# Hcyand/recommender_system

Hardware: AMD Instinct MI355X
Metric: CTR forward samples/sec @ batch 4096, 26 sparse×1e7 vocab, dim 16; %HBM roofline (higher is better)
Workload: dtype f32

## Files before the change

### recommender_system_amd/csrc/embed_fm_body.hpp

```cpp
#pragma once
#include "embed_fm.hpp"
#include "mlp_tower.hpp"

namespace rs {

#ifdef RS_DIAG_STAMPS
#define RS_STAMP(i)                                                                          \
  do {                                                                                       \
    __builtin_amdgcn_sched_barrier(0);                                                       \
    if (a.dbg && lane == 0)                                                                  \
      a.dbg[((int64_t)blockIdx.x * NW + w) * 16 + (i)] = __builtin_amdgcn_s_memrealtime();  \
    __builtin_amdgcn_sched_barrier(0);                                                       \
  } while (0)
#define RS_USE(x) asm volatile("" ::"v"(x))
#else
#define RS_STAMP(i) \
  do {              \
  } while (0)
#define RS_USE(x) \
  do {            \
  } while (0)
#endif

template <int KV, int NT, int NW, int KIND, bool TW, int MC = 0, bool PF = false, bool KA = false, int FC = 0,
          int KFMC = 0, int NDC = -1, bool PL = false>
__device__ __forceinline__ void embed_fm_body(const EmbedFmArgs& a, const MlpArgs* tw, const int tile,
                                              const FieldMeta* km = nullptr) {
  const int aF = FC > 0 ? FC : a.F;
  const int akfm = KFMC > 0 ? KFMC : a.kfm;
  const int and_ = NDC >= 0 ? NDC : a.nd;
  constexpr int MAXC0 = MC > 0 ? MC : 128 / (NW * KV);
  constexpr int MAXC = MAXC0 < 1 ? 1 : (MAXC0 > 8 ? 8 : MAXC0);
  typedef Ids<(KIND >= 3) ? 0 : KIND> I;
  constexpr bool OWNER = KIND == 4;
  __shared__ float cs[NW][16][NT * 16 + 1];
  __shared__ float qs[NW][16];

  const int lane = threadIdx.x & 63;
  const int w = __builtin_amdgcn_readfirstlane(threadIdx.x >> 6);
  const int s = lane & 15;
  const int kk = lane >> 4;
  const int64_t bt = (int64_t)tile * 16 + s;
  const bool valid = bt < a.batch;
  const int64_t b = bt < a.batch ? bt : a.batch - 1;
  const int d = and_ + aF * a.k;
  float w0v = (OWNER || PL) ? 0.f : a.w0[0];

  floatx4 ac[NT][4];
#pragma unroll
  for (int nt = 0; nt < NT; ++nt)
#pragma unroll
    for (int c = 0; c < 4; ++c) ac[nt][c] = floatx4{0.f, 0.f, 0.f, 0.f};
  float qn = 0.f;
  bool bad = false;

  if constexpr (!PL) {
    asm volatile("" ::"s"(a.ids), "s"(a.id_stride), "s"(a.dense), "s"(a.dense_stride), "s"(a.nd), "s"(a.table),
                 "s"(a.offs), "s"(a.vocab), "s"(aF), "s"(a.k), "s"(a.prep), "s"(akfm));
    asm volatile("" ::"s"(a.batch), "s"(a.DB), "s"(a.dense_rec), "s"(a.field_rec), "s"(a.field_base), "s"(a.x_out),
                 "s"(a.logit), "s"(a.w0), "s"(a.err));
  }
  RS_STAMP(0);
  RS_USE(b);
  RS_STAMP(5);
  if constexpr (TW) {
    const MlpArgs& a = *tw;
    MLP_STAMP(0);
  }
  extern __shared__ float tsm[];
  __shared__ float fmlog[TW ? 16 : 1];
  floatx4 ring[TW ? MLP_R : 1];
  const int xrs = TW ? tw->rs : 0;
  if constexpr (TW) {
    mlp_first_fill<NW>(*tw, ring);
    float* par = tsm + 32 * tw->rs + NW * 256;
    for (int i = threadIdx.x; i < tw->ptot; i += NW * 64) par[i] = tw->prep[tw->wtot + i];
    const int d0 = aF * a.k + and_, padw = tw->Kp[0] - d0;
    for (int i = threadIdx.x; i < 16 * padw; i += NW * 64) {
      const int r = i / padw;
      tsm[r * xrs + d0 + (i - r * padw)] = 0.f;
    }
  }
  const bool dense_small = KA || a.DB <= NW;
  const int dw = NW - 1 - w;
  const bool has_dense = dense_small && dw < a.DB;
  float dx = 0.f, dn = 0.f, drec[NT];
#pragma unroll
  for (int nt = 0; nt < NT; ++nt) drec[nt] = 0.f;
  auto load_dense = [&]() {
    if (has_dense) {
      const int e = 4 * dw + kk;
      dx = a.dense[b * a.dense_stride + (e < and_ ? e : 0)];
      const float* rec = a.prep + (int64_t)dw * a.dense_rec;
#pragma unroll
      for (int nt = 0; nt < NT; ++nt) drec[nt] = rec[nt * 64 + lane];
      dn = rec[NT * 64 + kk];
    }
  };
  constexpr int FMAX = 128;
  __shared__ typename I::raw_t lid[16][FMAX];
  __shared__ int64_t lmeta[2][FMAX];
#ifdef RS_DIAG_STAMPS
  const bool coop = !KA && !OWNER && (KIND != 3) && aF <= FMAX && !(a.ablate & 16);
#else
  const bool coop = !KA && !OWNER && (KIND != 3) && aF <= FMAX;
#endif
  if (coop) {
    const int64_t b0 = (int64_t)tile * 16;
    for (int t = threadIdx.x; t < 16 * aF; t += NW * 64) {
      const int ss = t / aF, c = t - ss * aF;
      const int64_t bb = b0 + ss < a.batch ? b0 + ss : a.batch - 1;
      const auto idv = I::load(a.ids, bb * a.id_stride + c);
#ifdef RS_DIAG_STAMPS
      RS_USE(idv);
      RS_STAMP(8);
#endif
      lid[ss][c] = idv;
    }
    if constexpr (!OWNER) {
      for (int t = threadIdx.x; t < 2 * aF; t += NW * 64) {
        const int c = t < aF ? t : t - aF;
        lmeta[t < aF ? 0 : 1][c] = t < aF ? a.offs[c] : a.vocab[c];
      }
    }
  }
  struct Pass {
    int cj[MAXC];
    bool ok[MAXC];
    typename I::raw_t rid[MAXC];
    int64_t off[MAXC], voc[MAXC];
    int64_t row[MAXC];
    Chunk<KV> xs[MAXC];
    Chunk<KV> bw[MAXC][NT];
    float nrm[MAXC][KV];
  };
  auto issue_b = [&](int cg, Pass& P) {
#pragma unroll
    for (int j = 0; j < MAXC; ++j) {
      const int c = cg + j * NW + w;
      P.cj[j] = c < aF ? c : aF - 1;
      const float* rec = a.prep + a.field_base + (int64_t)P.cj[j] * a.field_rec;
#pragma unroll
      for (int nt = 0; nt < NT; ++nt) {
#ifdef RS_DIAG_STAMPS
        if (a.ablate & 2) { P.bw[j][nt].zero(); P.bw[j][nt].v[0] = (float)P.cj[j]; continue; }
#endif
        if (nt * 16 + s <= akfm) P.bw[j][nt].load(rec + (int64_t)(nt * 64 + lane) * KV);
        else P.bw[j][nt].zero();
      }
    }
  };
  auto norms = [&](Pass& P) {
#pragma unroll
    for (int j = 0; j < MAXC; ++j)
#pragma unroll
      for (int tp = 0; tp < KV; ++tp) {
        float sq = 0.f;
#pragma unroll
        for (int nt = 0; nt < NT; ++nt) {
          const float bv = nt * 16 + s < akfm ? P.bw[j][nt].v[tp] : 0.f;
          sq = fmaf(bv, bv, sq);
        }
        P.nrm[j][tp] = row16_sum(sq);
      }
  };
  const int wv = threadIdx.x >> 6;
  auto fetch_ids = [&](int cg, Pass& P) {
    int64_t* offc = P.off;
    int64_t* vocc = P.voc;
#pragma unroll
    for (int j = 0; j < MAXC; ++j) {
      if constexpr (KIND != 3) {
        if (OWNER) {
          offc[j] = 0;
          vocc[j] = a.owner_rows;
          P.rid[j] = coop ? lid[s][P.cj[j]] : I::load(a.ids, b * a.id_stride + P.cj[j]);
        } else if (coop) {
          offc[j] = lmeta[0][P.cj[j]];
          vocc[j] = lmeta[1][P.cj[j]];
          P.rid[j] = lid[s][P.cj[j]];
        } else if constexpr (KA) {
          offc[j] = km->off[P.cj[j]];
          vocc[j] = km->voc[P.cj[j]];
          P.rid[j] = I::load(a.ids, b * a.id_stride + P.cj[j]);
        } else {
          const int cv = min(cg + j * NW + wv, aF - 1);
          offc[j] = a.offs[cv];
          vocc[j] = a.vocab[cv];
          P.rid[j] = I::load(a.ids, b * a.id_stride + P.cj[j]);
        }
      }
    }
    if (cg == 0 && !coop && aF > 0) load_dense();
  };
  auto decode_rows = [&](int cg, Pass& P) {
    if (cg == 0) RS_STAMP(6);
    else RS_STAMP(10);
#pragma unroll
    for (int j = 0; j < MAXC; ++j) {
      if constexpr (KIND == 3) {
        P.row[j] = b * aF + P.cj[j];
        P.ok[j] = true;
      } else {
        int64_t id;
        P.ok[j] = I::decode(P.rid[j], P.voc[j], id);
        P.row[j] = P.off[j] + id;
      }
    }
    RS_USE(P.row[MAXC - 1]);
    if (cg == 0) RS_STAMP(1);
    else RS_STAMP(11);
  };
  auto load_rows = [&](int cg, Pass& P) {
#pragma unroll
    for (int j = 0; j < MAXC; ++j) {
#ifdef RS_DIAG_STAMPS
      if ((a.ablate & 8) && cg + j * NW + w >= aF) { P.xs[j].zero(); continue; }
#endif
      P.xs[j].load_nt(a.table + P.row[j] * a.k + KV * kk);
    }
  };
  auto issue_rows = [&](int cg, Pass& P, bool fetched) {
    if (!fetched) fetch_ids(cg, P);
    decode_rows(cg, P);
    load_rows(cg, P);
  };
  auto consume = [&](int cg, Pass& P) {
    RS_USE(P.xs[MAXC - 1].v[KV - 1]);
    RS_USE(P.bw[MAXC - 1][0].v[KV - 1]);
    if (cg == 0) RS_STAMP(2);
    else RS_STAMP(12);
#pragma unroll
    for (int j = 0; j < MAXC; ++j) {
      const bool live = cg + j * NW + w < aF;
      if constexpr (OWNER) bad |= live && !P.ok[j] && P.rid[j] != -1;
      else bad |= live && !P.ok[j];
      const bool use = live && P.ok[j];
#pragma unroll
      for (int tp = 0; tp < KV; ++tp) {
        const float xv = use ? P.xs[j].v[tp] : 0.f;
#pragma unroll
        for (int nt = 0; nt < NT; ++nt) {
#ifdef RS_DIAG_STAMPS
          if (a.ablate & 1) { ac[nt][0][0] += xv * P.bw[j][nt].v[tp]; continue; }
#endif
          ac[nt][tp & 3] = mfma16x16x4(xv, P.bw[j][nt].v[tp], ac[nt][tp & 3]);
        }
        qn = fmaf(xv * xv, P.nrm[j][tp], qn);
      }
      if constexpr (TW) {
        if (live) {
          float* xo = tsm + s * xrs + P.cj[j] * a.k + KV * kk;
#pragma unroll
          for (int tp = 0; tp < KV; ++tp) xo[tp] = P.ok[j] ? P.xs[j].v[tp] : 0.f;
        }
      } else if (!KA && a.x_out && live && valid) {
        float* xo = a.x_out + b * d + and_ + P.cj[j] * a.k + KV * kk;
#pragma unroll
        for (int tp = 0; tp < KV; ++tp) xo[tp] = P.ok[j] ? P.xs[j].v[tp] : 0.f;
      }
    }
    RS_USE(ac[0][0][0]);
    if (cg == 0) RS_STAMP(13);
    else RS_STAMP(14);
  };
  auto has_pass = [&](int cg) { return cg < aF && !(MAXC == 1 && cg + w >= aF); };
  constexpr int PS = NW * MAXC;
  constexpr bool PRE = PF && KV * MAXC * NT <= 8;
  auto late_args = [&]() {
    if constexpr (PL) {
      w0v = a.w0[0];
      asm volatile("" ::"s"(a.k), "s"(a.logit), "s"(a.w0), "s"(a.err));
    }
  };
  Pass P0, P1;
  if (PRE) {
    if (has_pass(0)) issue_b(0, P0);
    if (has_pass(PS)) issue_b(PS, P1);
  }
  if (aF == 0 || coop) load_dense();
  if (coop) __syncthreads();
  RS_STAMP(9);
  if (PRE) {
    const bool one = has_pass(0), two = one && has_pass(PS);
    if (one) {
      fetch_ids(0, P0);
      if (two) fetch_ids(PS, P1);
    } else if (!coop && aF > 0) {
      load_dense();
    }
    late_args();
    if (one) {
      issue_rows(0, P0, true);
      if constexpr (PL) asm volatile("" ::"s"(w0v));
      norms(P0);
      if (two) norms(P1);
      if (two) decode_rows(PS, P1);
      consume(0, P0);
      if (two) {
        load_rows(PS, P1);
        consume(PS, P1);
        for (int cg = 2 * PS; !KA && has_pass(cg); cg += PS) {
          issue_b(cg, P0);
          issue_rows(cg, P0, false);
          norms(P0);
          consume(cg, P0);
        }
      }
    }
  } else {
    late_args();
    for (int cg = 0; has_pass(cg); cg += PS) {
      issue_b(cg, P0);
      issue_rows(cg, P0, false);
      norms(P0);
      consume(cg, P0);
    }
  }

  if (has_dense) {
    const int e = 4 * dw + kk;
    dx = e < and_ ? dx : 0.f;
#pragma unroll
    for (int nt = 0; nt < NT; ++nt) ac[nt][0] = mfma16x16x4(dx, drec[nt], ac[nt][0]);
    qn = fmaf(dx * dx, dn, qn);
    if constexpr (TW) {
      if (e < and_) tsm[s * xrs + aF * a.k + e] = dx;
    } else if (!KA && a.x_out && valid && e < and_) {
      a.x_out[b * d + e] = dx;
    }
  }
  if (!dense_small) {
    for (int t = w; t < a.DB; t += NW) {
      const int e = 4 * t + kk;
      const float xv = a.dense[b * a.dense_stride + (e < and_ ? e : 0)];
      const float x = e < and_ ? xv : 0.f;
      const float* rec = a.prep + (int64_t)t * a.dense_rec;
#pragma unroll
      for (int nt = 0; nt < NT; ++nt) ac[nt][0] = mfma16x16x4(x, rec[nt * 64 + lane], ac[nt][0]);
      qn = fmaf(x * x, rec[NT * 64 + kk], qn);
      if constexpr (TW) {
        if (e < and_) tsm[s * xrs + aF * a.k + e] = x;
      } else if (a.x_out && valid && e < and_) {
        a.x_out[b * d + e] = x;
      }
    }
  }
  floatx4 acc[NT];
#pragma unroll
  for (int nt = 0; nt < NT; ++nt)
#pragma unroll
    for (int i = 0; i < 4; ++i) acc[nt][i] = (ac[nt][0][i] + ac[nt][1][i]) + (ac[nt][2][i] + ac[nt][3][i]);
  RS_USE(acc[0][0]);
  RS_STAMP(3);
  if (__any(bad && valid) && lane == 0) flag_error(a.err);

#ifdef RS_DIAG_STAMPS
  if (a.ablate & 4) {
    if (w == 0 && kk == 0 && b < a.batch) a.logit[b] = acc[0][0] + acc[0][1] + qn;
    return;
  }
#endif
#pragma unroll
  for (int nt = 0; nt < NT; ++nt)
#pragma unroll
    for (int r = 0; r < 4; ++r) cs[w][kk * 4 + r][nt * 16 + s] = acc[nt][r];
  qn += __shfl_xor(qn, 16);
  qn += __shfl_xor(qn, 32);
  if (lane < 16) qs[w][lane] = qn;
  __syncthreads();
  RS_STAMP(7);
  constexpr int NC = NT * 16;
  if (threadIdx.x < 16 * NC) {
    const int smp = threadIdx.x / NC, col = threadIdx.x % NC;
    float v = 0.f;
#pragma unroll
    for (int ww = 0; ww < NW; ++ww) v += cs[ww][smp][col];
    float t = col < akfm ? v * v : 0.f;
    if (col < NW) t -= qs[col][smp];
    float lin = col == akfm ? v : 0.f;
    t = row16_sum(t);
    lin = row16_sum(lin);
    if constexpr (NT == 2) {
      t += __shfl_xor(t, 16);
      lin += __shfl_xor(lin, 16);
    }
    const int64_t bb = (int64_t)tile * 16 + smp;
    if constexpr (OWNER) {
      float q = col < NW ? qs[col][smp] : 0.f;
      q = row16_sum(q);
      if constexpr (NT == 2) q += __shfl_xor(q, 16);
      if (bb < a.batch) {
        float* rec = a.logit + bb * a.pstride;
        if (col <= akfm) rec[col] = v;
        if (col == 0) rec[akfm + 1] = q;
        else if (akfm + 1 + col < a.pw) rec[akfm + 1 + col] = 0.f;
      }
      return;
    }
    const float fm = (lin + w0v) + 0.5f * t;
    if (col == 0 && bb < a.batch && a.logit) a.logit[bb] = fm;
    if constexpr (TW) {
      if (col == 0) fmlog[smp] = fm;
    }
  }
  RS_STAMP(4);
  if constexpr (TW) {
    {
      const MlpArgs& a = *tw;
      MLP_STAMP(1);
    }
    mlp_tower_tile<NW>(*tw, tsm, (int64_t)tile * 16, ring, fmlog);
  }
}

struct EmbedFmCold {
  float* logit;
  const float* w0;
  int* err;
  int F, k, nd, kfm;
  const int64_t* offs;
  const int64_t* vocab;
  float* x_out;
  int DB;
  int64_t dense_rec, field_rec, field_base;
  int64_t owner_rows;
  int pw;
  int64_t pstride;
  unsigned long long* dbg;
  int ablate;
};

static inline EmbedFmCold cold_args(const EmbedFmArgs& a) {
  return EmbedFmCold{a.logit, a.w0,        a.err,       a.F,          a.k,          a.nd, a.kfm,     a.offs, a.vocab,
                     a.x_out, a.DB,        a.dense_rec, a.field_rec,  a.field_base, a.owner_rows,    a.pw,   a.pstride,
                     a.dbg,   a.ablate};
}

template <int KV, int NT, int FC, int KFMC, int NDC>
__device__ __forceinline__ EmbedFmArgs hot_cold_args(const float* prep, const void* ids, int64_t id_stride,
                                                     int64_t batch, const float* dense, int64_t dense_stride,
                                                     const float* table, const EmbedFmCold& c) {
  EmbedFmArgs a;
  a.ids = ids;
  a.id_stride = id_stride;
  a.dense = dense;
  a.dense_stride = dense_stride;
  a.nd = c.nd;
  a.table = table;
  a.offs = c.offs;
  a.vocab = c.vocab;
  a.F = c.F;
  a.k = c.k;
  a.prep = prep;
  a.w0 = c.w0;
  a.kfm = c.kfm;
  a.logit = c.logit;
  a.x_out = c.x_out;
  a.batch = batch;
  a.err = c.err;
  if constexpr (FC > 0) {
    constexpr FmGeom G = fm_geom(NDC, FC, 4 * KV, KFMC);
    static_assert(G.mfma && G.KV == KV && G.NT == NT, "specialised shape: not this instantiation's geometry");
    a.DB = G.DB;
    a.dense_rec = G.dense_rec;
    a.field_rec = G.field_rec;
    a.field_base = G.field_base;
  } else {
    a.DB = c.DB;
    a.dense_rec = c.dense_rec;
    a.field_rec = c.field_rec;
    a.field_base = c.field_base;
  }
  a.owner_rows = c.owner_rows;
  a.pw = c.pw;
  a.pstride = c.pstride;
  a.dbg = c.dbg;
  a.ablate = c.ablate;
  return a;
}

}
```

Before: 713.0 million.

## Restructure FM embed body: early second-pass row loads, wide LDS reduce, permlane swaps

Several independent tweaks to the fused embedding+FM kernel. A compile-time row stride is used when the field count is fixed. The second pass's row offsets are precomputed and its table loads are issued behind a scheduling barrier before the first pass is consumed, to overlap gather latency. Dense loading moves out of fetch_ids when prefetching, and the per-field bias loads become unconditional in the KA path. The cross-wave LDS reduction layout is transposed so each output reads contiguous floatx4 vectors, and qn shuffles are replaced with permlane16/32 swaps. Together these add code complexity and raise register pressure and LDS size.

Measured after the change: 751.6 million, median of 6. 1.05x the previous value.

```diff
diff --git a/recommender_system_amd/csrc/embed_fm_body.hpp b/recommender_system_amd/csrc/embed_fm_body.hpp
--- a/recommender_system_amd/csrc/embed_fm_body.hpp
+++ b/recommender_system_amd/csrc/embed_fm_body.hpp
@@ -33,17 +33,22 @@
   constexpr int MAXC = MAXC0 < 1 ? 1 : (MAXC0 > 8 ? 8 : MAXC0);
   typedef Ids<(KIND >= 3) ? 0 : KIND> I;
   constexpr bool OWNER = KIND == 4;
-  __shared__ float cs[NW][16][NT * 16 + 1];
+  constexpr int NC = NT * 16;
+  constexpr bool WIDE = !TW && NW % 4 == 0;
+  constexpr int CW = NW + 4;
+  __shared__ __attribute__((aligned(16))) float cs[WIDE ? 16 * NC * CW : NW * 16 * (NC + 1)];
   __shared__ float qs[NW][16];
 
   const int lane = threadIdx.x & 63;
   const int w = __builtin_amdgcn_readfirstlane(threadIdx.x >> 6);
   const int s = lane & 15;
   const int kk = lane >> 4;
+  const int ak = FC > 0 ? 4 * KV : a.k;
   const int64_t bt = (int64_t)tile * 16 + s;
   const bool valid = bt < a.batch;
-  const int64_t b = bt < a.batch ? bt : a.batch - 1;
-  const int d = and_ + aF * a.k;
+  const int64_t b = (KA && !TW) ? (int64_t)(uint32_t)(valid ? (int)bt : (int)a.batch - 1)
+                                : (bt < a.batch ? bt : a.batch - 1);
+  const int d = and_ + aF * ak;
   float w0v = (OWNER || PL) ? 0.f : a.w0[0];
 
   floatx4 ac[NT][4];
@@ -75,7 +80,7 @@
     mlp_first_fill<NW>(*tw, ring);
     float* par = tsm + 32 * tw->rs + NW * 256;
     for (int i = threadIdx.x; i < tw->ptot; i += NW * 64) par[i] = tw->prep[tw->wtot + i];
-    const int d0 = aF * a.k + and_, padw = tw->Kp[0] - d0;
+    const int d0 = aF * ak + and_, padw = tw->Kp[0] - d0;
     for (int i = threadIdx.x; i < 16 * padw; i += NW * 64) {
       const int r = i / padw;
       tsm[r * xrs + d0 + (i - r * padw)] = 0.f;
@@ -145,7 +150,7 @@
 #ifdef RS_DIAG_STAMPS
         if (a.ablate & 2) { P.bw[j][nt].zero(); P.bw[j][nt].v[0] = (float)P.cj[j]; continue; }
 #endif
-        if (nt * 16 + s <= akfm) P.bw[j][nt].load(rec + (int64_t)(nt * 64 + lane) * KV);
+        if (KA || nt * 16 + s <= akfm) P.bw[j][nt].load(rec + (int64_t)(nt * 64 + lane) * KV);
         else P.bw[j][nt].zero();
       }
     }
@@ -164,6 +169,8 @@
         P.nrm[j][tp] = row16_sum(sq);
       }
   };
+  constexpr int PS = NW * MAXC;
+  constexpr bool PRE = PF && KV * MAXC * NT <= 8;
   const int wv = threadIdx.x >> 6;
   auto fetch_ids = [&](int cg, Pass& P) {
     int64_t* offc = P.off;
@@ -191,7 +198,7 @@
         }
       }
     }
-    if (cg == 0 && !coop && aF > 0) load_dense();
+    if (!PRE && cg == 0 && !coop && aF > 0) load_dense();
   };
   auto decode_rows = [&](int cg, Pass& P) {
     if (cg == 0) RS_STAMP(6);
@@ -217,7 +224,7 @@
 #ifdef RS_DIAG_STAMPS
       if ((a.ablate & 8) && cg + j * NW + w >= aF) { P.xs[j].zero(); continue; }
 #endif
-      P.xs[j].load_nt(a.table + P.row[j] * a.k + KV * kk);
+      P.xs[j].load_nt(a.table + P.row[j] * ak + KV * kk);
     }
   };
   auto issue_rows = [&](int cg, Pass& P, bool fetched) {
@@ -250,12 +257,12 @@
       }
       if constexpr (TW) {
         if (live) {
-          float* xo = tsm + s * xrs + P.cj[j] * a.k + KV * kk;
+          float* xo = tsm + s * xrs + P.cj[j] * ak + KV * kk;
 #pragma unroll
           for (int tp = 0; tp < KV; ++tp) xo[tp] = P.ok[j] ? P.xs[j].v[tp] : 0.f;
         }
       } else if (!KA && a.x_out && live && valid) {
-        float* xo = a.x_out + b * d + and_ + P.cj[j] * a.k + KV * kk;
+        float* xo = a.x_out + b * d + and_ + P.cj[j] * ak + KV * kk;
 #pragma unroll
         for (int tp = 0; tp < KV; ++tp) xo[tp] = P.ok[j] ? P.xs[j].v[tp] : 0.f;
       }
@@ -265,40 +272,60 @@
     else RS_STAMP(14);
   };
   auto has_pass = [&](int cg) { return cg < aF && !(MAXC == 1 && cg + w >= aF); };
-  constexpr int PS = NW * MAXC;
-  constexpr bool PRE = PF && KV * MAXC * NT <= 8;
   auto late_args = [&]() {
     if constexpr (PL) {
       w0v = a.w0[0];
-      asm volatile("" ::"s"(a.k), "s"(a.logit), "s"(a.w0), "s"(a.err));
+      if constexpr (FC == 0) asm volatile("" ::"s"(a.k));
+      asm volatile("" ::"s"(a.logit), "s"(a.w0), "s"(a.err));
     }
   };
   Pass P0, P1;
+  const bool one = FC >= NW || has_pass(0), two = has_pass(PS);
   if (PRE) {
-    if (has_pass(0)) issue_b(0, P0);
-    if (has_pass(PS)) issue_b(PS, P1);
+    if (one) issue_b(0, P0);
+    if (two) issue_b(PS, P1);
   }
   if (aF == 0 || coop) load_dense();
   if (coop) __syncthreads();
   RS_STAMP(9);
   if (PRE) {
-    const bool one = has_pass(0), two = one && has_pass(PS);
     if (one) {
       fetch_ids(0, P0);
       if (two) fetch_ids(PS, P1);
-    } else if (!coop && aF > 0) {
-      load_dense();
-    }
+    }
+    if (!coop && aF > 0) load_dense();
     late_args();
     if (one) {
       issue_rows(0, P0, true);
       if constexpr (PL) asm volatile("" ::"s"(w0v));
       norms(P0);
       if (two) norms(P1);
-      if (two) decode_rows(PS, P1);
+      int64_t ro[MAXC];
+#pragma unroll
+      for (int j = 0; j < MAXC; ++j) ro[j] = 0;
+      if (two) {
+        decode_rows(PS, P1);
+#pragma unroll
+        for (int j = 0; j < MAXC; ++j) {
+          ro[j] = P1.row[j] * ak + KV * kk;
+          asm volatile("" : "+v"(ro[j]));
+        }
+      }
+      asm volatile("" ::"v"(P0.xs[MAXC - 1].v[KV - 1]));
+      __builtin_amdgcn_sched_barrier(0);
+      if (two) {
+#pragma unroll
+        for (int j = 0; j < MAXC; ++j) {
+#ifdef RS_DIAG_STAMPS
+          if ((a.ablate & 8) && PS + j * NW + w >= aF) { P1.xs[j].zero(); continue; }
+#endif
+          P1.xs[j].load_nt(a.table + ro[j]);
+        }
+        RS_STAMP(15);
+      }
+      __builtin_amdgcn_sched_barrier(0);
       consume(0, P0);
       if (two) {
-        load_rows(PS, P1);
         consume(PS, P1);
         for (int cg = 2 * PS; !KA && has_pass(cg); cg += PS) {
           issue_b(cg, P0);
@@ -325,7 +352,7 @@
     for (int nt = 0; nt < NT; ++nt) ac[nt][0] = mfma16x16x4(dx, drec[nt], ac[nt][0]);
     qn = fmaf(dx * dx, dn, qn);
     if constexpr (TW) {
-      if (e < and_) tsm[s * xrs + aF * a.k + e] = dx;
+      if (e < and_) tsm[s * xrs + aF * ak + e] = dx;
     } else if (!KA && a.x_out && valid && e < and_) {
       a.x_out[b * d + e] = dx;
     }
@@ -340,7 +367,7 @@
       for (int nt = 0; nt < NT; ++nt) ac[nt][0] = mfma16x16x4(x, rec[nt * 64 + lane], ac[nt][0]);
       qn = fmaf(x * x, rec[NT * 64 + kk], qn);
       if constexpr (TW) {
-        if (e < and_) tsm[s * xrs + aF * a.k + e] = x;
+        if (e < and_) tsm[s * xrs + aF * ak + e] = x;
       } else if (a.x_out && valid && e < and_) {
         a.x_out[b * d + e] = x;
       }
@@ -364,18 +391,32 @@
 #pragma unroll
   for (int nt = 0; nt < NT; ++nt)
 #pragma unroll
-    for (int r = 0; r < 4; ++r) cs[w][kk * 4 + r][nt * 16 + s] = acc[nt][r];
-  qn += __shfl_xor(qn, 16);
-  qn += __shfl_xor(qn, 32);
+    for (int r = 0; r < 4; ++r) {
+      const int smp = kk * 4 + r, col = nt * 16 + s;
+      cs[WIDE ? (smp * NC + col) * CW + w : (w * 16 + smp) * (NC + 1) + col] = acc[nt][r];
+    }
+  __builtin_amdgcn_sched_barrier(0);
+  const auto h = __builtin_amdgcn_permlane16_swap(__float_as_uint(qn), __float_as_uint(qn), false, false);
+  qn = __uint_as_float(h[0]) + __uint_as_float(h[1]);
+  const auto f = __builtin_amdgcn_permlane32_swap(__float_as_uint(qn), __float_as_uint(qn), false, false);
+  qn = __uint_as_float(f[0]) + __uint_as_float(f[1]);
   if (lane < 16) qs[w][lane] = qn;
   __syncthreads();
   RS_STAMP(7);
-  constexpr int NC = NT * 16;
   if (threadIdx.x < 16 * NC) {
     const int smp = threadIdx.x / NC, col = threadIdx.x % NC;
     float v = 0.f;
-#pragma unroll
-    for (int ww = 0; ww < NW; ++ww) v += cs[ww][smp][col];
+    if constexpr (WIDE) {
+      const floatx4* pw = reinterpret_cast<const floatx4*>(cs + (smp * NC + col) * CW);
+      floatx4 pv[NW / 4];
+#pragma unroll
+      for (int g = 0; g < NW / 4; ++g) pv[g] = pw[g];
+#pragma unroll
+      for (int ww = 0; ww < NW; ++ww) v += pv[ww / 4][ww % 4];
+    } else {
+#pragma unroll
+      for (int ww = 0; ww < NW; ++ww) v += cs[(ww * 16 + smp) * (NC + 1) + col];
+    }
     float t = col < akfm ? v * v : 0.f;
     if (col < NW) t -= qs[col][smp];
     float lin = col == akfm ? v : 0.f;
```
